# DataCanvasIO/DeepTables

Measured on AMD Instinct MI355X. Metric: training rows/sec (fwd+bwd) DeepFM Criteo-shape batch 8192, higher is better.
Workload: dtype f32 (split-bf16: 24-bit fwd / 16-bit bwd)

## Files before the change

__graft_entry__.py:

```python
import glob
import hashlib
import os
import subprocess
import sys

ROOT = os.path.dirname(os.path.abspath(__file__))
CSRC = os.path.join(ROOT, 'deeptables_amd', 'csrc')
LIB = os.path.join(ROOT, 'deeptables_amd', 'libdt_hip.so')


def _sources():
    return sorted(glob.glob(os.path.join(CSRC, '*.hip')) + glob.glob(os.path.join(CSRC, '*.cpp')))


def _deps():
    return _sources() + sorted(glob.glob(os.path.join(CSRC, '*.h'))) + [os.path.join(ROOT, 'include', 'dt_hip.h')]


def source_hash():
    h = hashlib.sha256()
    for p in _deps():
        h.update(os.path.basename(p).encode())
        h.update(open(p, 'rb').read())
    return h.hexdigest()[:16]


def _loaded_hash():
    if not os.path.exists(LIB):
        return None
    code = ('import ctypes,sys; l=ctypes.CDLL(sys.argv[1]); f=l.dt_source_hash; f.restype=ctypes.c_char_p; '
            'print(f().decode())')
    try:
        return subprocess.check_output([sys.executable, '-c', code, LIB], stderr=subprocess.DEVNULL,
                                       timeout=60).decode().strip()
    except Exception:
        return None


def _compile_one(args):
    hipcc, src, obj, want = args
    cmd = [hipcc, '--offload-arch=gfx950', '-O3', '-std=c++17', '-fPIC', '-Wno-unused-value',
           f'-DDT_SOURCE_HASH="{want}"' if src.endswith('lib.cpp') else '-DDT_UNUSED', '-x', 'hip', '-c', src, '-o', obj]
    subprocess.check_call(cmd)
    return obj


def build(force=False):
    want = source_hash()
    have = None if force else _loaded_hash()
    if have != want:
        hipcc = os.environ.get('HIPCC', '/opt/rocm/bin/hipcc')
        if not os.path.exists(hipcc):
            raise RuntimeError(f'hipcc not found and the in-tree libdt_hip.so ({have}) does not match the sources ({want})')
        bdir = os.path.join(CSRC, '_build')
        os.makedirs(bdir, exist_ok=True)
        common = hashlib.sha256()
        for p in _deps():
            if p.endswith('.h'):
                common.update(open(p, 'rb').read())
        jobs, objs = [], []
        for src in _sources():
            key = hashlib.sha256(common.digest() + open(src, 'rb').read() +
                                 (want.encode() if src.endswith('lib.cpp') else b'')).hexdigest()[:16]
            obj = os.path.join(bdir, os.path.basename(src) + '.' + key + '.o')
            objs.append(obj)
            if force or not os.path.exists(obj):
                for old in glob.glob(os.path.join(bdir, os.path.basename(src) + '.*.o')):
                    os.remove(old)
                jobs.append((hipcc, src, obj, want))
        print(f'[build] hipcc --offload-arch=gfx950 -O3: {len(jobs)} of {len(objs)} objects to compile')
        if jobs:
            from concurrent.futures import ThreadPoolExecutor
            with ThreadPoolExecutor(max_workers=min(len(jobs), os.cpu_count() or 4)) as ex:
                list(ex.map(_compile_one, jobs))
        subprocess.check_call([hipcc, '--offload-arch=gfx950', '-shared', '-fPIC'] + objs + ['-o', LIB + '.tmp'])
        os.replace(LIB + '.tmp', LIB)
    if ROOT not in sys.path:
        sys.path.insert(0, ROOT)
    import deeptables_amd
    from deeptables_amd import _lib
    h = _lib.lib()
    assert h.dt_version() == 1 and h.dt_build_arch() == b'gfx950'
    got = h.dt_source_hash().decode()
    assert got == want, f'libdt_hip.so was built from other sources: {got} != {want}'
    print('[build] ok:', LIB, 'exports', len(_lib.SIGNATURES), 'entry points; source hash', got,
          '(rebuilt)' if have != want else '(binary matches the sources)')


def smoke():
    if ROOT not in sys.path:
        sys.path.insert(0, ROOT)
    build()
    import torch
    assert torch.cuda.is_available(), 'smoke() needs a GPU'
    from deeptables_amd import functional, ops
    from deeptables_amd.models import ModelConfig, DeepModel, deepnets
    from deeptables_amd.models.metainfo import CategoricalColumn, ContinuousColumn
    from oracle import bridge, reference_layers as R
    dev = torch.device('cuda', 0)
    F, Nd, D, B, V = 26, 13, 16, 256, 1000
    functional.set_seed(7)
    conf = ModelConfig(nets=deepnets.DeepFM, fixed_embedding_dim=True, embeddings_output_dim=D,
                       embedding_dropout=0, metrics=['AUC'])
    cats = [CategoricalColumn(f'C{i}', V, D) for i in range(F)]
    conts = [ContinuousColumn('input_continuous_all', [f'I{j}' for j in range(Nd)])]
    dm = DeepModel('binary', 2, conf, cats, conts)
    dm.build(dev)
    g = torch.Generator().manual_seed(1)
    idx = torch.randint(0, V, (B, F), generator=g)
    dense = torch.randn(B, Nd, generator=g)
    y = (torch.rand(B, 1, generator=g) < 0.25).float()
    ref_logit, _ = bridge.oracle_forward(dm, idx, dense, training=True)
    dm.model.train()
    emb_layer = dm.model.layers_by_name['emb_categorical_vars_all']
    emb, _ = ops.embedding_lookup(idx.int().to(dev), emb_layer.tables['d16'], emb_layer.row_offset_d16,
                                  emb_layer.vocab_d16)
    ref_emb = torch.cat(R.multi_column_embedding(idx.float(), [e.detach().cpu() for e in emb_layer.embeddings]), 1)
    assert torch.equal(emb.detach().cpu(), ref_emb), 'embedding gather is not bit-exact'
    loss, logit = dm.train_step([idx.int().to(dev), dense.to(dev)], y.to(dev))
    torch.cuda.synchronize()
    err = (logit.double().cpu() - ref_logit).abs().max().item()
    print(f'[smoke] DeepFM B={B}: loss={float(loss):.6f}  max|logit - oracle|={err:.2e}  gather bit-exact')
    assert err < 1e-4, f'logit mismatch vs oracle: {err}'


if __name__ == '__main__':
    build(force='--force' in sys.argv)
    if '--smoke' in sys.argv:
        smoke()
```

deeptables_amd/csrc/deepfm.hip:

```cpp
#include <stdlib.h>
#include "common.h"
#include "adam_dev.h"

namespace dt {

typedef float floatx16 __attribute__((ext_vector_type(16)));
typedef float floatx4_t __attribute__((ext_vector_type(4)));

constexpr int kH1 = 128;
constexpr int kH2 = 64;
constexpr int kTM = 32;

struct DeepFmDims {
    int B, F, D, Nd, C, CP;
};

struct DeepFmAccum {
    int64_t dW1, dW2, db1, db2, dw3, dwo, dbo, loss, dgamma, dbeta, dwlin, slin, total;
    int64_t dw3d, dcw, dcb, sumc, sumcx;
};
__host__ __device__ inline DeepFmAccum deepfm_accum_layout(int C, int CP, int F, int Nd, int L = 0) {
    DeepFmAccum a;
    int64_t o = 0;
    a.dW1 = o; o += (int64_t)C * kH1;
// ... 1771 lines not shown
#pragma unroll
            for (int pt = 0; pt < 2; ++pt) {
                lay.W2R[pt * lay.w2r_lo + (int64_t)k0 * kH2 + n] = q0[pt];
                lay.W2R[pt * lay.w2r_lo + (int64_t)(k0 + 1) * kH2 + n] = q1[pt];
            }
        }
        return;
    }
    const float dg = wave_sum(w.x * m.x + w.y * m.y);
    const float db = wave_sum(w.x * d.x + w.y * d.y);
    const float ga_b = ga, be_b = be;
    {
        const floatx2 g = floatx2{ga * m.x + be * d.x, ga * m.y + be * d.y};
        *reinterpret_cast<floatx2*>(accum + e0) = g;
        if (da.p) adam2(g.x, g.y);
        if (da.p && lay.W1B) {
            __bf16 q0[3], q1[3];
            x3_parts(pnew[0], q0);
            x3_parts(pnew[1], q1);
            const int k = col, n0 = 2 * lane;
            const int64_t kb = ((int64_t)(k >> 5) * 8) * 64 * 8 + (((k >> 3) & 3) * 16) * 8 + (k & 7);
            const int64_t i0 = kb + ((int64_t)(n0 >> 4) * 64 + (n0 & 15)) * 8, i1 = kb + ((int64_t)((n0 + 1) >> 4) * 64 + ((n0 + 1) & 15)) * 8;
#pragma unroll
            for (int pt = 0; pt < 3; ++pt) {
                lay.W1B[pt * lay.w1b_lo + i0] = q0[pt];
                lay.W1B[pt * lay.w1b_lo + i1] = q1[pt];
            }
#pragma unroll
            for (int pt = 0; pt < 2; ++pt) {
                typedef __bf16 b2 __attribute__((ext_vector_type(2)));
                *reinterpret_cast<b2*>(lay.W1R + pt * lay.w1r_lo + (int64_t)k * kH1 + n0) = b2{q0[pt], q1[pt]};
            }
        }
    }
    if (Lc) {
        const int scal = pl.cross + (Lc + 1) * dm.CP;
        const int l = lane;
        const float sa_mine = l < Lc ? rec_sum(rs, scal + 16 + l) : 0.f;
        const float sco_mine = l <= Lc ? rec_sum(rs, scal + l) : 0.f;
        const float G = l <= Lc ? gp.gsum[(int64_t)l * dm.CP + col] : 0.f;
        const float sdz = rec_sum(rs, scal + 31);
        float cl = 0.f, suf = 0.f;
        for (int j = 0; j < Lc; ++j) {
            const float saj = __shfl(sa_mine, j, 64);
            const float bj = cb[(int64_t)j * dm.C + col], wj = cw[(int64_t)j * dm.C + col];
            if (j < l) cl += bj;
            if (j > l) suf += saj * wj;
        }
        if (l <= Lc) {
            const int64_t ig = l < Lc ? al.dcw + (int64_t)l * dm.C + col : al.dw3 + col;
            const float gw = ga_b * G + be_b * sco_mine + (l < Lc ? sa_mine : sdz) * cl;
            const float gb = sdz * w3c[col] + suf;
            accum[ig] = gw;
            if (l < Lc) accum[al.dcb + (int64_t)l * dm.C + col] = gb;
            if (da.p) {
                adam_one(da.p, da.m, da.v, ig, gw, da.lr_t, da.b1, da.b2, da.eps);
                if (l < Lc) adam_one(da.p, da.m, da.v, al.dcb + (int64_t)l * dm.C + col, gb, da.lr_t, da.b1, da.b2, da.eps);
                if (lay.cwp) {
                    lay.cwp[(int64_t)(l < Lc ? l : 2 * Lc) * dm.CP + col] = da.p[ig];
                    if (l < Lc) lay.cwp[(int64_t)(Lc + l) * dm.CP + col] = da.p[al.dcb + (int64_t)l * dm.C + col];
                }
            }
        }
    }
}

__global__ __launch_bounds__(256) void k_bn_grads2(const float* __restrict__ W1, const float* __restrict__ gamma,
                                                   const float* __restrict__ beta, DeepFmDims dm, float* accum,
                                                   DeepFmAccum al, const float* __restrict__ wpart, int row_blocks,
                                                   int Lc, const float* __restrict__ cw, const float* __restrict__ cb,
                                                   const float* __restrict__ w3c, RecSrc rs, int col_blocks, GPart gp) {
    __shared__ floatx2 sm[4][64];
    __shared__ float slin_s[kMaxC];
    const DenseAdam none{nullptr, nullptr, nullptr, 0.f, 0.f, 0.f, 0.f};
    const Part3 pl = part3_layout(dm.CP, Lc, 1);
    if ((int)blockIdx.x < col_blocks)
        bn_grads2_body(W1, gamma, beta, dm, accum, al, wpart, row_blocks, Lc, cw, cb, w3c, rs, pl, sm, slin_s, none, (int)blockIdx.x, gp);
    else
        finish_record_entry(((int)blockIdx.x - col_blocks) * (int)blockDim.x + (int)threadIdx.x, rs, pl, al, dm, Lc, accum, none);
}

__global__ __launch_bounds__(256) void k_finish_records(DeepFmDims dm, float* accum, DeepFmAccum al, int Lc, RecSrc rs,
                                                        double* __restrict__ bnacc_zero, int bnacc_n) {
    const DenseAdam none{nullptr, nullptr, nullptr, 0.f, 0.f, 0.f, 0.f};
    const Part3 pl = part3_layout(dm.CP, Lc, 0);
    const int i = (int)blockIdx.x * (int)blockDim.x + (int)threadIdx.x;
    finish_record_entry(i, rs, pl, al, dm, Lc, accum, none);
    for (int j = i; j < bnacc_n; j += (int)(gridDim.x * blockDim.x)) bnacc_zero[j] = 0.0;
}

struct FinishSeg {
    SegTail seg;
    float *table, *m, *v;
    const float* values;
    int sstride, D;
};
__global__ __launch_bounds__(256) void k_finish_step(const float* __restrict__ W1, const float* __restrict__ gamma,
                                                     const float* __restrict__ beta, DeepFmDims dm, float* accum,
                                                     DeepFmAccum al, const float* __restrict__ wpart, int row_blocks,
                                                     DenseAdam da, AdamState* __restrict__ st, float lr, int col_blocks,
                                                     int small_blocks, int seg_blocks, FinishSeg fs, int Lc,
                                                     const float* __restrict__ cw, const float* __restrict__ cb,
                                                     const float* __restrict__ w3c, RecSrc rs, X3Lay lay, GPart gp,
                                                     const float* __restrict__ lr_snap) {
    __shared__ floatx2 sm[4][64];
    __shared__ float slin_s[kMaxC];
    const Part3 pl = part3_layout(dm.CP, Lc, 1);
    const int sb = (int)blockIdx.x < seg_blocks ? (int)blockIdx.x : -1;
    const int b = sb >= 0 ? col_blocks + small_blocks : (int)blockIdx.x - seg_blocks < small_blocks
                      ? col_blocks + ((int)blockIdx.x - seg_blocks) : (int)blockIdx.x - seg_blocks - small_blocks;
    int nseg0 = 0;
    if (sb >= 0 && fs.seg.nseg) nseg0 = fs.seg.nseg[(sb * (int)(blockDim.x >> 6) + (int)(threadIdx.x >> 6)) % fs.seg.regions];
    if (lr_snap) da.lr_t = *lr_snap; else if (st) da.lr_t = st->lr_t;
    if (b < col_blocks) {
        bn_grads2_body(W1, gamma, beta, dm, accum, al, wpart, row_blocks, Lc, cw, cb, w3c, rs, pl, sm, slin_s, da, b, gp, lay);
    } else if (b < col_blocks + small_blocks) {
        finish_record_entry((b - col_blocks) * (int)blockDim.x + (int)threadIdx.x, rs, pl, al, dm, Lc, accum, da);
    } else if (fs.seg.nseg) {
        adam_segments<true>(fs.seg, seg_blocks, nseg0, fs.table, fs.m, fs.v, fs.values, fs.D, da.lr_t, da.b1, da.b2, da.eps,
                      fs.sstride, sb);
    }
    if (lr_snap) {
        if (blockIdx.x == 0 && threadIdx.x == 0 && st) {
            const int t = st->t + 1;
            st->t = t;
            st->lr_t = adam_lr_t(lr, da.b1, da.b2, t);
        }
    } else {
        __syncthreads();
        adam_finish(st, threadIdx.x == 0 ? 0u : kNoTicket, lr, da.b1, da.b2);
    }
}

__global__ void k_emb_drop_advance(unsigned* seed) { *seed = *seed * 1664525u + 1013904223u; }

struct RowsAdam {
    float *table, *m, *v;
    int sstride;
    const float* lr_t_dev;
    float lr_t_host, b1, b2, eps;
    int wt;
};
struct RowsEpi {
    const float *dXn, *X, *dz, *S, *wlin, *sc, *mean, *rstd;
    RecSrc rs;
    int sdx, sdxx;
    const int64_t* rows_out;
    float* grad_rows;
    float grad_scale;
    int field_major;
};
constexpr int kRowsUB = 4;

template <bool DCN>
__device__ __forceinline__ void rows_epilogue_wave(unsigned* work, int first_tile, int tile_stride, const DeepFmDims& dm,
                                                   const RowsEpi& a, const RowsAdam& ad, const EmbDrop& drop) {
    const int lane = threadIdx.x & 63, wv = threadIdx.x >> 6;
    const int LPR = dm.D >> 2, TPR = dm.F * LPR;
    const int parts = TPR > 64 ? 2 : 1;
    const int lpp = (TPR + parts - 1) / parts;
    const int rpw = parts == 1 ? 64 / TPR : 1;
    const int part = wv & (parts - 1);
    const int rsub = lane / lpp, pl = lane - rsub * lpp;
    const int piece = min(part * lpp + pl, TPR - 1);
    const bool active = rsub < rpw && part * lpp + pl < TPR;
    const int f = piece / LPR, c = piece - f * LPR;
    const int col = 4 * piece;
    const int tiles = (dm.B + kTM - 1) / kTM;
    const int chunk_rows = rpw * kRowsUB, chunks = (kTM + chunk_rows - 1) / chunk_rows;
    int dshift = 0;
    while ((1 << dshift) < dm.D) ++dshift;
    const floatx4 ca = ld4(a.sc + col), cmu = ld4(a.mean + col);
    floatx4 c1, c2;
    {
        typedef double doublex2 __attribute__((ext_vector_type(2)));
        doublex2 s1[2] = {{0.0, 0.0}, {0.0, 0.0}}, s2[2] = {{0.0, 0.0}, {0.0, 0.0}};
#pragma unroll
        for (int sh = 0; sh < kRecShards; ++sh) {
            const double* q = a.rs.racc + (int64_t)sh * a.rs.stride;
            s1[0] += *reinterpret_cast<const doublex2*>(q + a.sdx + col);
            s1[1] += *reinterpret_cast<const doublex2*>(q + a.sdx + col + 2);
            s2[0] += *reinterpret_cast<const doublex2*>(q + a.sdxx + col);
            s2[1] += *reinterpret_cast<const doublex2*>(q + a.sdxx + col + 2);
        }
        const floatx4 rsd = ld4(a.rstd + col);
        const float invN = 1.0f / (float)dm.B;
        c1 = floatx4{(float)s1[0][0], (float)s1[0][1], (float)s1[1][0], (float)s1[1][1]} * invN;
        c2 = rsd * floatx4{(float)s2[0][0], (float)s2[0][1], (float)s2[1][0], (float)s2[1][1]} * invN;
    }
    const float wl = DCN ? 0.f : a.wlin[f];
    const float lr_t = ad.lr_t_dev ? *ad.lr_t_dev : ad.lr_t_host;
    const unsigned dseed = drop.thr ? *drop.seed : 0u;
    for (;;) {
        unsigned it = 0;
        if (lane == 0) it = atomicAdd(&work[part], 1u);
        it = __builtin_amdgcn_readfirstlane(it);
        const int ti = (int)(it / (unsigned)chunks), ch = (int)(it - (unsigned)ti * (unsigned)chunks);
        const int tile = first_tile + ti * tile_stride;
        if (tile >= tiles) break;
        const int b0 = tile * kTM;
        {
            int64_t row[kRowsUB];
            floatx4 gx[kRowsUB], xr[kRowsUB], sv[kRowsUB];
            float dzv[kRowsUB];
            bool ok[kRowsUB];
            int bb[kRowsUB];
#pragma unroll
            for (int k = 0; k < kRowsUB; ++k) {
                const int r = ch * chunk_rows + k * rpw + rsub;
                ok[k] = active && r < kTM && b0 + r < dm.B;
                bb[k] = min(b0 + min(r, kTM - 1), dm.B - 1);
                row[k] = a.rows_out[(int64_t)bb[k] * dm.F + f];
            }
#pragma unroll
            for (int k = 0; k < kRowsUB; ++k) {
                gx[k] = ld4(a.dXn + (int64_t)bb[k] * dm.CP + col);
                xr[k] = ld4(a.X + (int64_t)bb[k] * dm.CP + col);
                if (!DCN) {
                    sv[k] = ld4(a.S + ((int64_t)bb[k] << dshift) + 4 * c);
                    dzv[k] = a.dz[bb[k]];
                }
            }
            floatx4 pv[kRowsUB], mv[kRowsUB], vv[kRowsUB];
            bool upd[kRowsUB];
#pragma unroll
            for (int k = 0; k < kRowsUB; ++k) {
                upd[k] = ok[k] && ad.table && row[k] >= 0;
                if (ad.table) {
                    const int64_t rr = upd[k] ? row[k] : 0;
                    pv[k] = drop.thr ? ld4(ad.table + (rr << dshift) + 4 * c) : xr[k];
                    mv[k] = ld4(ad.m + rr * ad.sstride + 4 * c);
                    vv[k] = ld4(ad.v + rr * ad.sstride + 4 * c);
                }
            }
#pragma unroll
            for (int k = 0; k < kRowsUB; ++k) {
                floatx4 g = ca * (gx[k] - c1 - (xr[k] - cmu) * c2);
                if (!DCN) g = g + dzv[k] * wl + dzv[k] * (sv[k] - xr[k]);
                if (drop.thr) {
                    float4 t4 = make_float4(g.x, g.y, g.z, g.w);
                    t4 = emb_drop4(t4, dseed, drop.thr, drop.inv_keep, (unsigned)bb[k], (unsigned)col);
                    g = floatx4{t4.x, t4.y, t4.z, t4.w};
                }
                if (upd[k]) {
                    floatx4 mi = mv[k], vi = vv[k], pi = pv[k];
#pragma unroll
                    for (int e = 0; e < 4; ++e) {
                        mi[e] = ad.b1 * mi[e] + (1.f - ad.b1) * g[e];
                        vi[e] = ad.b2 * vi[e] + (1.f - ad.b2) * g[e] * g[e];
                        pi[e] -= lr_t * mi[e] / (sqrtf(vi[e]) + ad.eps);
                    }
                    st4_sel(ad.m + row[k] * ad.sstride + 4 * c, mi, ad.wt);
                    st4_sel(ad.v + row[k] * ad.sstride + 4 * c, vi, ad.wt);
                    st4_sel(ad.table + (row[k] << dshift) + 4 * c, pi, ad.wt);
                } else if (ok[k]) {
                    if (a.field_major)
                        st4(a.grad_rows + (((int64_t)f * dm.B + bb[k]) << dshift) + 4 * c, g * a.grad_scale);
                    else
                        st4(a.grad_rows + (((int64_t)bb[k] * dm.F + f) << dshift) + 4 * c, g);
                }
            }
        }
    }
}

template <bool DCN, int WM = 0>
__global__ __launch_bounds__(512) void k_wgrad_rows(const float* __restrict__ X, MlpParams p, DeepFmDims dm,
                                                    const float* __restrict__ H1, const float* __restrict__ dH1,
                                                    const float* __restrict__ dH2, int row_blocks, int rows_per_block,
                                                    float* __restrict__ wpart, unsigned long long* stamps_all,
                                                    RowsEpi ep, RowsAdam ad, EmbDrop drop,
                                                    unsigned long long* stamps_rows, int matrix_waves_join,
                                                    double* __restrict__ bnacc_zero, int bnacc_n, StepNext nx, GPart gp,
                                                    float* __restrict__ lr_snap) {
    extern __shared__ __attribute__((aligned(16))) float red[];
    __shared__ unsigned arrived, work[2], ecnt;
    if (threadIdx.x == 0) { arrived = 0u; work[0] = 0u; work[1] = 0u; ecnt = 0u; }
    __syncthreads();
    if (threadIdx.x < 256) {
        if constexpr (WM == 0)
            wgrad_heavy(red, (int)blockIdx.x, X, p, dm, H1, dH1, dH2, row_blocks, rows_per_block, wpart, stamps_all, &arrived);
        else
            wgrad_heavy_bf16<WM>(red, (int)blockIdx.x, X, p, dm, H1, dH1, dH2, row_blocks, rows_per_block, wpart, &arrived);
        ElectSync sy{&ecnt, 0u};
        if (DCN && gp.part) reduce_gpart(gp, red, (int)blockIdx.x, (int)gridDim.x, (int)threadIdx.x, sy);
        if (nx.idx) {
            for (int e = (int)blockIdx.x; e < nx.eblocks; e += (int)gridDim.x) {
                elect_barrier<256, true>(sy);
                elect_block<256, true, 32>(reinterpret_cast<unsigned long long*>(red), nx.dd, dm.B, dm.F, e, (int)threadIdx.x,
                                           nx.rows_out, sy);
            }
        }
        if (matrix_waves_join) rows_epilogue_wave<DCN>(work, (int)blockIdx.x, (int)gridDim.x, dm, ep, ad, drop);
        if (stamps_all && threadIdx.x == 0) stamps_all[(int64_t)blockIdx.x * 16 + 6] = __builtin_amdgcn_s_memtime();
    } else {
        if (stamps_rows && threadIdx.x == 256) stamps_rows[(int64_t)blockIdx.x * 16] = __builtin_amdgcn_s_memtime();
        for (int j = (int)blockIdx.x * 256 + ((int)threadIdx.x - 256); j < bnacc_n; j += (int)gridDim.x * 256) bnacc_zero[j] = 0.0;
        if (lr_snap && blockIdx.x == 0 && threadIdx.x == 256) *lr_snap = ad.lr_t_dev ? *ad.lr_t_dev : ad.lr_t_host;
        rows_epilogue_wave<DCN>(work, (int)blockIdx.x, (int)gridDim.x, dm, ep, ad, drop);
        if (stamps_rows && threadIdx.x == 256) stamps_rows[(int64_t)blockIdx.x * 16 + 3] = __builtin_amdgcn_s_memtime();
    }
}

}

using namespace dt;

static bool deepfm_dims(int B, int F, int D, int Nd, DeepFmDims* dm, int* lpr) {
    if (B <= 0 || F <= 0 || D <= 0 || Nd < 0 || D % 4) return false;
    const int l = D / 4;
    if (l < 1 || l > 64 || (l & (l - 1))) return false;
    if (F * l > 128 || Nd > 64) return false;
    dm->B = B; dm->F = F; dm->D = D; dm->Nd = Nd;
    dm->C = F * D + Nd;
    dm->CP = (dm->C + 63) & ~63;
    if (dm->C > 544 || D > 64) return false;
    *lpr = l;
    return true;
}

extern "C" int dt_deepfm_supported(int B, int F, int D, int Nd, int H1, int H2) {
    DeepFmDims dm; int lpr;
    return (H1 == kH1 && H2 == kH2 && deepfm_dims(B, F, D, Nd, &dm, &lpr)) ? 1 : 0;
}

struct DeepFmWs {
    int64_t X, H1, dH1, dH2, lin, fm, z, dz, dlogit, mean, rstd, sc, betap, W1L, W2L, W2TL, S, wpart, bnacc, racc, stamps, dXc, dXn,
        gammap, x3, total;
    int64_t bnacc_n, racc_n;
    int64_t gpart, gsum;
    int64_t lrsnap;
};
static DeepFmWs deepfm_ws_layout(const DeepFmDims& dm, int L = 0) {
    DeepFmWs w;
    int64_t o = 0;
    auto take = [&](int64_t n) { int64_t r = o; o += (n + 3) & ~(int64_t)3; return r; };
    const int tiles = ceil_div(dm.B, kTM);
    const int64_t rows = (int64_t)tiles * kTM;
    w.X = take(rows * dm.CP);
    w.H1 = take(rows * kH1);
    w.dH1 = take(rows * kH1);
    w.dH2 = take(rows * kH2);
    w.lin = take(rows); w.fm = take(rows); w.z = take(rows); w.dz = take(rows); w.dlogit = take(rows);
    w.mean = take(dm.CP); w.rstd = take(dm.CP); w.sc = take(dm.CP); w.betap = take(dm.CP);
    w.W1L = take((int64_t)dm.CP * kH1);
    w.W2L = take((int64_t)kH1 * kH2);
    w.W2TL = take((int64_t)kH1 * kH2);
    w.S = take(rows * dm.D);
    w.wpart = take((int64_t)256 * 8192);
    w.bnacc_n = (int64_t)kBnShards * 2 * dm.CP;
    w.bnacc = take(2 * w.bnacc_n);
    w.racc_n = (int64_t)kRecShards * part3_layout(dm.CP, L, 1).stride;
    w.racc = take(2 * w.racc_n);
    w.gpart = take(L > 0 ? (int64_t)tiles * (L + 1) * dm.CP : 0);
    w.gsum = take(L > 0 ? (int64_t)(L + 1) * dm.CP : 0);
    w.stamps = take((int64_t)5 * tiles * 16 * 2);
    w.dXc = take(L > 0 ? rows * dm.CP : 0);
    w.dXn = take(rows * dm.CP);
    w.gammap = take(dm.CP);
    w.lrsnap = take(4);
    w.x3 = take((5 * (int64_t)dm.CP * kH1 + 5 * (int64_t)kH1 * kH2 + 1) / 2 + (2 * kCrossMax + 1) * (int64_t)dm.CP);
    w.total = o;
    return w;
}

extern "C" int64_t dt_deepfm_workspace_bytes(int B, int F, int D, int Nd) {
    DeepFmDims dm; int lpr;
    if (!deepfm_dims(B, F, D, Nd, &dm, &lpr)) return -1;
    return deepfm_ws_layout(dm).total * (int64_t)sizeof(float);
}

extern "C" int64_t dt_deepfm_stamps_offset_floats(int B, int F, int D, int Nd) {
    DeepFmDims dm; int lpr;
    if (!deepfm_dims(B, F, D, Nd, &dm, &lpr)) return -1;
    return deepfm_ws_layout(dm).stamps;
}

extern "C" int64_t dt_deepfm_accum_floats(int F, int D, int Nd) {
    const int C = F * D + Nd, CP = (C + 63) & ~63;
    return deepfm_accum_layout(C, CP, F, Nd).total;
}

extern "C" int dt_deepfm_accum_offsets(int F, int D, int Nd, int64_t* out11) {
    const int C = F * D + Nd, CP = (C + 63) & ~63;
    const DeepFmAccum a = deepfm_accum_layout(C, CP, F, Nd);
    const int64_t v[11] = {a.dW1, a.dW2, a.db1, a.db2, a.dw3, a.dwo, a.dbo, a.loss, a.dgamma, a.dbeta, a.dwlin};
    for (int i = 0; i < 11; ++i) out11[i] = v[i];
    return DT_OK;
}

extern "C" unsigned dt_deepfm_dropout_hash(unsigned seed, unsigned b, unsigned col) { return emb_drop_hash(seed, b, col); }

extern "C" int64_t dt_deepfm_dedupe_slots(int B, int F) {
    return (int64_t)B * F;
}

struct DedupeLayout {
    int64_t rows_fm, nseg, seg_row, seg_off, seg_cnt, seg_list, list_cur, overflow, pid, total;
    int pid_stride;
    int eblocks, parts_log2;
    int regions, cap;
    bool by_field;
};
static DedupeLayout dedupe_layout(int B, int F) {
    const int64_t n = (int64_t)B * F;
    DedupeLayout l;
    l.by_field = B > kElectSlots;
    l.parts_log2 = 0;
    while (((l.by_field ? 4096 : 1024) << l.parts_log2) < B) ++l.parts_log2;
    const int fpad = ((F + 7) >> 3) << 3;
    l.eblocks = fpad << l.parts_log2;
    l.regions = l.by_field ? fpad : l.eblocks;
    l.cap = l.by_field ? (B >> 1) : kSegCap;
    int64_t o = 0;
    auto take = [&](int64_t bytes) { int64_t r = o; o += (bytes + 15) & ~(int64_t)15; return r; };
    l.rows_fm = take(n * 8); l.nseg = take((int64_t)l.regions * 4);
    l.seg_row = take((int64_t)l.regions * l.cap * 8); l.seg_off = take((int64_t)l.regions * l.cap * 4);
    l.seg_cnt = take((int64_t)l.regions * l.cap * 4); l.seg_list = take((int64_t)l.regions * B * 4);
    l.list_cur = take((int64_t)fpad * 4);
    l.overflow = take(16);
    l.pid_stride = (B + 15) & ~15;
    l.pid = take(l.by_field ? (int64_t)fpad * l.pid_stride : 0);
    l.total = o;
    return l;
}
static DedupeWs dedupe_view(void* dedupe_ws, const DedupeLayout& dl) {
    char* base = reinterpret_cast<char*>(dedupe_ws);
    DedupeWs dd{reinterpret_cast<int64_t*>(base + dl.rows_fm), dl.parts_log2, reinterpret_cast<int*>(base + dl.nseg),
                reinterpret_cast<int64_t*>(base + dl.seg_row), reinterpret_cast<int*>(base + dl.seg_off),
                reinterpret_cast<int*>(base + dl.seg_cnt), reinterpret_cast<int*>(base + dl.seg_list),
                dl.by_field ? reinterpret_cast<int*>(base + dl.nseg) : nullptr,
                dl.by_field ? reinterpret_cast<int*>(base + dl.list_cur) : nullptr,
                reinterpret_cast<int*>(base + dl.overflow),
                dl.by_field ? reinterpret_cast<unsigned char*>(base + dl.pid) : nullptr, dl.pid_stride};
    return dd;
}

extern "C" int64_t dt_deepfm_dedupe_bytes(int B, int F) { return dedupe_layout(B, F).total; }

extern "C" int dt_deepfm_dedupe_segments(int B, int F, int64_t* out7) {
    const DedupeLayout l = dedupe_layout(B, F);
    out7[0] = l.nseg; out7[1] = l.seg_row; out7[2] = l.seg_off; out7[3] = l.seg_cnt; out7[4] = l.seg_list;
    out7[5] = l.regions; out7[6] = l.cap;
    return DT_OK;
}

extern "C" int64_t dt_deepfm_dedupe_overflow_offset(int B, int F) { return dedupe_layout(B, F).overflow; }

extern "C" int dt_deepfm_preelect(const void* idx, int idx_kind, const int64_t* row_offset, const int32_t* vocab, int B,
                                  int F, int64_t* rows_out, void* dedupe_ws, int64_t dedupe_slots, void* stream) {
    DT_REQUIRE(idx && row_offset && vocab && rows_out && dedupe_ws && B > 0 && F > 0 && F <= 128,
               "dt_deepfm_preelect: bad arguments");
// ... 639 lines not shown
```

deeptables_amd/csrc/tower_x3.h:

```cpp
#pragma once

typedef __bf16 x3_b8 __attribute__((ext_vector_type(8)));
typedef __bf16 x3_b4 __attribute__((ext_vector_type(4)));

struct X3Weights {
    const __bf16* W1B; int64_t w1b_lo;
    const __bf16* W1R; int64_t w1r_lo;
    const __bf16* W2B; int64_t w2b_lo;
    const __bf16* W2R; int64_t w2r_lo;
    const float* cwp;
};

__device__ __forceinline__ void x3_split2(const float (&v)[8], x3_b8& h, x3_b8& l) {
#pragma unroll
    for (int e = 0; e < 8; ++e) {
        const __bf16 a = (__bf16)v[e];
        h[e] = a;
        l[e] = (__bf16)(v[e] - (float)a);
    }
}
__device__ __forceinline__ void x3_split3(const float (&v)[8], x3_b8& h, x3_b8& m, x3_b8& l) {
#pragma unroll
    for (int e = 0; e < 8; ++e) {
        const __bf16 a = (__bf16)v[e];
// ... 25 lines not shown
}

template <int NCH, int LC = 0, bool ONE = false>
__global__ __launch_bounds__(512) void k_tower_x3(const float* __restrict__ X, MlpParams p, X3Weights xw, DeepFmDims dm,
                                                  const float* __restrict__ lin, const float* __restrict__ fm,
                                                  const float* __restrict__ y, float* __restrict__ H1,
                                                  float* __restrict__ dH1, float* __restrict__ dH2,
                                                  float* __restrict__ z_out, float* __restrict__ logit_out,
                                                  float* __restrict__ dlogit, float* __restrict__ dz_out,
                                                  double* __restrict__ part, unsigned long long* stamps, DcnArgs dc,
                                                  float* __restrict__ dxn_out) {
    extern __shared__ __attribute__((aligned(16))) float lds[];
    DT_STAMP(stamps, 0);
    constexpr int CP = 64 * NCH, NST = CP / 32, XSB = CP + 16, XS = CP + 4, HF = kH1 + 4, DF = kH2 + 4;
    constexpr int XP = kTM * XSB;
    char* base = reinterpret_cast<char*>(lds);
    __bf16* xb = reinterpret_cast<__bf16*>(base);
    float* xs = reinterpret_cast<float*>(base);
    float* slp = xs + kTM * XS;
    float* zp = slp + 8 * CP;
    float* dzs = zp + 4 * kTM;
    float* cs = dzs + kTM;
    float* bnp = reinterpret_cast<float*>(base + (size_t)3 * XP * 2);
    float* h1f = bnp + 4 * CP;
    float* d2f = h1f + kTM * HF;
    float* pb = d2f + kTM * DF;
    float* crP = pb + 2 * 48 * 16;
    float* crA = crP + 48 * 16;
    float* crF = crA + kTM * 16;
    float* zcs = crF + kTM * 16;
    const int tid = threadIdx.x, lane = tid & 63, wave = tid >> 6;
    const int n16 = lane & 15, kg = lane >> 4;
    const int m0 = blockIdx.x * kTM;
    const Part3 pl = part3_layout(dm.CP, LC ? dc.L : 0, 1);
    double* prec = part + (int64_t)((int)blockIdx.x & (kRecShards - 1)) * pl.stride;

    const int srow = tid >> 4, qcol = 4 * (tid & 15);
    const int bcol = min(tid, dm.C - 1);
    double bsx[kBnShards], bsq[kBnShards];
#pragma unroll
    for (int w = 0; w < kBnShards; ++w) {
        bsx[w] = p.bnacc[(int64_t)w * 2 * dm.CP + bcol];
        bsq[w] = p.bnacc[(int64_t)w * 2 * dm.CP + dm.CP + bcol];
    }
    const float gam = p.gamma[bcol], bet = p.beta[bcol];
    floatx4 xv[NCH];
#pragma unroll
    for (int j = 0; j < NCH; ++j) xv[j] = ld4(X + (int64_t)(m0 + srow) * CP + 64 * j + qcol);
    constexpr int kPF = 5;
    const __bf16* w1b = xw.W1B + ((int64_t)wave * 64 + lane) * 8;
    x3_b8 bq[kPF][3];
#pragma unroll
    for (int s = 0; s < kPF; ++s)
#pragma unroll
        for (int q = 0; q < 3; ++q) bq[s][q] = x3_ld8(w1b + q * xw.w1b_lo + (int64_t)(s < NST ? s : 0) * 4096);
    const int mt2 = wave & 1, nt2 = wave >> 1;
    const float bias1 = p.b1[16 * wave + n16];
    const float b2v = p.b2[16 * nt2 + n16], w3v = p.w3[16 * nt2 + n16];
    float linv = 0.f, fmv = 0.f, yv = 0.f, wov = 0.f, bov = 0.f, swv = 1.f;
    const float invB = 1.0f / (float)dm.B;
    const double invBd = 1.0 / (double)dm.B;
    if (wave == 0) {
        wov = p.wo[0];
        bov = p.bo ? p.bo[0] : 0.f;
        if (lane < 32 && m0 + lane < dm.B) {
            if (LC == 0) { linv = lin[m0 + lane]; fmv = fm[m0 + lane]; }
            yv = y[m0 + lane];
            if (dc.sw) swv = dc.sw[m0 + lane];
        }
    }
    DT_STAMP(stamps, 6);
    {
        const int col = tid;
        float mean = 0.f, sc = 0.f, be = 0.f, rstd = 0.f, var = 0.f;
        if (col < dm.C) {
            double sx = 0.0, sq = 0.0;
#pragma unroll
            for (int w = 0; w < kBnShards; ++w) { sx += bsx[w]; sq += bsq[w]; }
            const double md = sx * invBd, vd = sq * invBd - md * md;
            mean = (float)md;
            var = vd > 0.0 ? (float)vd : 0.f;
            rstd = 1.0f / sqrtf(var + p.eps);
            sc = rstd * gam;
            be = bet;
        }
        if (col < CP) {
            bnp[col] = mean; bnp[CP + col] = sc; bnp[2 * CP + col] = be; bnp[3 * CP + col] = rstd;
            if (blockIdx.x == 0) {
                p.mean_w[col] = mean; p.rstd_w[col] = rstd; p.sc_w[col] = sc; p.betap_w[col] = be;
                p.gammap_w[col] = col < dm.C ? gam : 0.f;
                if (col < dm.C) {
                    if (p.moving_mean) p.moving_mean[col] = p.moving_mean[col] * p.momentum + mean * (1.f - p.momentum);
                    if (p.moving_var) p.moving_var[col] = p.moving_var[col] * p.momentum + var * (1.f - p.momentum);
                }
            }
        }
    }
    static_assert(CP <= 512, "one column per thread in the BN prologue");
    lds_barrier();
    DT_STAMP(stamps, 7);
#pragma unroll
    for (int j = 0; j < NCH; ++j) {
        const floatx4 mu = ld4(bnp + 64 * j + qcol), sc = ld4(bnp + CP + 64 * j + qcol), be = ld4(bnp + 2 * CP + 64 * j + qcol);
        const floatx4 xn = (xv[j] - mu) * sc + be;
        x3_b4 h, m, l;
#pragma unroll
        for (int e = 0; e < 4; ++e) {
            const __bf16 a = (__bf16)xn[e];
            const float r1 = xn[e] - (float)a;
            const __bf16 b = (__bf16)r1;
            h[e] = a; m[e] = b; l[e] = (__bf16)(r1 - (float)b);
        }
        __bf16* dst = xb + srow * XSB + 64 * j + qcol;
        *reinterpret_cast<x3_b4*>(dst) = h;
        *reinterpret_cast<x3_b4*>(dst + XP) = m;
        *reinterpret_cast<x3_b4*>(dst + 2 * XP) = l;
    }
    lds_barrier();
    DT_STAMP(stamps, 1);

    x3_b8 w2q[4][3];
    float h1r[2][4];
    {
        floatx4 c1[2], c2[2], c3[2];
#pragma unroll
        for (int t = 0; t < 2; ++t) { c1[t] = floatx4{0.f, 0.f, 0.f, 0.f}; c2[t] = c1[t]; c3[t] = c1[t]; }
        const __bf16* arow0 = xb + n16 * XSB + 8 * kg;
        const __bf16* arow1 = xb + (16 + n16) * XSB + 8 * kg;
        x3_b8 an[2][3];
#pragma unroll
        for (int q = 0; q < 3; ++q) { an[0][q] = x3_ld8(arow0 + q * XP); an[1][q] = x3_ld8(arow1 + q * XP); }
#pragma unroll
        for (int s = 0; s < NST; ++s) {
            x3_b8 a[2][3], b[3];
#pragma unroll
            for (int q = 0; q < 3; ++q) { a[0][q] = an[0][q]; a[1][q] = an[1][q]; b[q] = bq[s % kPF][q]; }
            if (s + 1 < NST) {
#pragma unroll
                for (int q = 0; q < 3; ++q) {
                    an[0][q] = x3_ld8(arow0 + q * XP + 32 * (s + 1));
                    an[1][q] = x3_ld8(arow1 + q * XP + 32 * (s + 1));
                }
            }
            if (s + kPF < NST) {
#pragma unroll
                for (int q = 0; q < 3; ++q) bq[s % kPF][q] = x3_ld8(w1b + q * xw.w1b_lo + (int64_t)(s + kPF) * 4096);
            }
            if (NST >= 4 && s >= NST - 4) {
                const int g = s - (NST - 4);
                const __bf16* w2b = xw.W2B + (((int64_t)g * 4 + nt2) * 64 + lane) * 8;
#pragma unroll
                for (int q = 0; q < 3; ++q) w2q[g][q] = x3_ld8(w2b + q * xw.w2b_lo);
            }
            X3_MFMA(c1[0], a[0][0], b[0]); X3_MFMA(c1[1], a[1][0], b[0]);
            X3_LO(c2[0], a[0][0], b[1]); X3_LO(c2[1], a[1][0], b[1]);
            X3_LO(c3[0], a[0][0], b[2]); X3_LO(c3[1], a[1][0], b[2]);
            X3_LO(c2[0], a[0][1], b[0]); X3_LO(c2[1], a[1][1], b[0]);
            X3_LO(c3[0], a[0][1], b[1]); X3_LO(c3[1], a[1][1], b[1]);
            X3_LO(c3[0], a[0][2], b[0]); X3_LO(c3[1], a[1][2], b[0]);
        }
        if constexpr (NST < 4) {
#pragma unroll
            for (int g = 0; g < 4; ++g) {
                const __bf16* w2b = xw.W2B + (((int64_t)g * 4 + nt2) * 64 + lane) * 8;
#pragma unroll
                for (int q = 0; q < 3; ++q) w2q[g][q] = x3_ld8(w2b + q * xw.w2b_lo);
            }
        }
        DT_STAMP(stamps, 2);
        if constexpr (LC > 0) {
            if (wave < 6) {
                const int L = dc.L, mt = wave % 3, kh = wave / 3;
                const int s0 = kh * (NST / 2), s1 = kh ? NST : NST / 2;
                const float* brow = xw.cwp + (int64_t)(n16 < L ? n16 : 2 * L) * CP + 8 * kg;
                const float bmask = n16 <= L ? 1.f : 0.f;
                const float* arow2 = xw.cwp + (int64_t)(L + min(n16, L - 1)) * CP + 8 * kg;
                const float amask2 = n16 < L ? 1.f : 0.f;
                floatx4 q1 = {0.f, 0.f, 0.f, 0.f}, q2 = q1, q3 = q1;
                for (int st = s0; st < s1; ++st) {
                    float bv[8];
                    x3_ld8f(brow + 32 * st, bv);
#pragma unroll
                    for (int e = 0; e < 8; ++e) bv[e] *= bmask;
                    x3_b8 b1, b2, b3, a1, a2, a3;
                    x3_split3(bv, b1, b2, b3);
                    if (mt < 2) {
                        const __bf16* ap = xb + (16 * mt + n16) * XSB + 32 * st + 8 * kg;
                        a1 = x3_ld8(ap); a2 = x3_ld8(ap + XP); a3 = x3_ld8(ap + 2 * XP);
                    } else {
                        float av[8];
                        x3_ld8f(arow2 + 32 * st, av);
#pragma unroll
                        for (int e = 0; e < 8; ++e) av[e] *= amask2;
                        x3_split3(av, a1, a2, a3);
                    }
                    X3_MFMA(q3, a1, b3); X3_MFMA(q3, a2, b2); X3_MFMA(q3, a3, b1);
                    X3_MFMA(q2, a1, b2); X3_MFMA(q2, a2, b1);
                    X3_MFMA(q1, a1, b1);
                }
#pragma unroll
                for (int r = 0; r < 4; ++r) pb[(kh * 48 + 16 * mt + 4 * kg + r) * 16 + n16] = (q3[r] + q2[r]) + q1[r];
            }
        }
#pragma unroll
        for (int t = 0; t < 2; ++t)
#pragma unroll
            for (int r = 0; r < 4; ++r) {
                const float h = fmaxf(((c3[t][r] + c2[t][r]) + c1[t][r]) + bias1, 0.f);
                h1r[t][r] = h;
                h1f[(16 * t + 4 * kg + r) * HF + 16 * wave + n16] = h;
            }
    }
    x3_b8 w2r[2][2];
#pragma unroll
    for (int g = 0; g < 2; ++g) {
        const __bf16* src = xw.W2R + (int64_t)(16 * wave + n16) * kH2 + 32 * g + 8 * kg;
        w2r[g][0] = x3_ld8(src); w2r[g][1] = x3_ld8(src + xw.w2r_lo);
    }
    lds_barrier();
    DT_STAMP(stamps, 3);

    float h2r[4];
    {
        floatx4 c1 = {0.f, 0.f, 0.f, 0.f}, c2 = c1, c3 = c1;
        const float* arow = h1f + (16 * mt2 + n16) * HF + 8 * kg;
        floatx4 hrow[2];
#pragma unroll
        for (int u = 0; u < 2; ++u) hrow[u] = ld4(h1f + ((tid >> 5) + 16 * u) * HF + 4 * (tid & 31));
#pragma unroll
        for (int g = 0; g < 4; ++g) {
            float v[8];
            x3_ld8f(arow + 32 * g, v);
            x3_b8 a1, a2, a3;
            x3_split3(v, a1, a2, a3);
            X3_MFMA(c1, a1, w2q[g][0]);
            X3_LO(c2, a1, w2q[g][1]);
            X3_LO(c3, a1, w2q[g][2]);
            X3_LO(c2, a2, w2q[g][0]);
            X3_LO(c3, a2, w2q[g][1]);
            X3_LO(c3, a3, w2q[g][0]);
        }
#pragma unroll
        for (int u = 0; u < 2; ++u) {
            const int m = m0 + (tid >> 5) + 16 * u;
            if (m < dm.B) st4_sel(H1 + (int64_t)m * kH1 + 4 * (tid & 31), hrow[u], dc.wt);
        }
        float zr[4];
#pragma unroll
        for (int r = 0; r < 4; ++r) {
            h2r[r] = fmaxf(((c3[r] + c2[r]) + c1[r]) + b2v, 0.f);
            zr[r] = group_sum<16>(h2r[r] * w3v);
        }
        if (n16 == 0) {
#pragma unroll
            for (int r = 0; r < 4; ++r) zp[nt2 * kTM + 16 * mt2 + 4 * kg + r] = zr[r];
        }
    }
#pragma unroll
    for (int j = 0; j < NCH; ++j) {
        const floatx4 mu = ld4(bnp + 64 * j + qcol), rs = ld4(bnp + 3 * CP + 64 * j + qcol);
        st4(xs + srow * XS + 64 * j + qcol, (xv[j] - mu) * rs);
    }
    if constexpr (LC > 0) {
        for (int e = tid; e < 48 * 16; e += 512) crP[e] = pb[e] + pb[48 * 16 + e];
    }
    lds_barrier();
    DT_STAMP(stamps, 4);
    const int NT = (dm.C + 15) >> 4;
    auto w1r = [&](int nt) {
        const int col = min(16 * nt + n16, CP - 1);
        return xw.W1R + (int64_t)col * kH1 + 8 * kg;
    };
    x3_b8 bW[2][4][2];
#pragma unroll
    for (int i = 0; i < 2; ++i) {
        if (wave + 8 * i < NT) {
            const __bf16* wr = w1r(wave + 8 * i);
#pragma unroll
            for (int g = 0; g < 4; ++g) { bW[i][g][0] = x3_ld8(wr + 32 * g); bW[i][g][1] = x3_ld8(wr + xw.w1r_lo + 32 * g); }
        }
    }

    if (wave == 0) {
        const int c = lane & 31, s = lane >> 5;
        const int m = m0 + c;
        float zc = 0.f;
        if constexpr (LC > 0) {
            const int L = dc.L;
            static_assert(LC + 1 <= 12, "three float4 per row of crP");
            float pr[12], gq[LC][12];
            {
                const floatx4 t0 = ld4(crP + c * 16), t1 = ld4(crP + c * 16 + 4), t2 = ld4(crP + c * 16 + 8);
#pragma unroll
                for (int e = 0; e < 4; ++e) { pr[e] = t0[e]; pr[4 + e] = t1[e]; pr[8 + e] = t2[e]; }
            }
#pragma unroll
            for (int j = 0; j < LC; ++j) {
                const floatx4 t0 = ld4(crP + (32 + j) * 16), t1 = ld4(crP + (32 + j) * 16 + 4), t2 = ld4(crP + (32 + j) * 16 + 8);
#pragma unroll
                for (int e = 0; e < 4; ++e) { gq[j][e] = t0[e]; gq[j][4 + e] = t1[e]; gq[j][8 + e] = t2[e]; }
            }
            float a = 1.f;
#pragma unroll
            for (int l = 0; l <= LC; ++l) {
                float q = 0.f;
#pragma unroll
// ... 45 lines not shown

    {
        float sb = 0.f, sw = 0.f;
#pragma unroll
        for (int r = 0; r < 4; ++r) {
            const int row = 16 * mt2 + 4 * kg + r;
            const float dzv = dzs[row];
            const float g = h2r[r] > 0.f ? dzv * w3v : 0.f;
            d2f[row * DF + 16 * nt2 + n16] = g;
            sb += g;
            sw += dzv * h2r[r];
        }
        sb = row_pair16(sb, false); sw = row_pair16(sw, false);
        if (kg == 0) { cs[(mt2 * 2 + 0) * kH2 + 16 * nt2 + n16] = sb; cs[(mt2 * 2 + 1) * kH2 + 16 * nt2 + n16] = sw; }
        if constexpr (LC == 0) {
            const float dzr = dzs[srow];
#pragma unroll
            for (int j = 0; j < NCH; ++j) {
                floatx4 v = xv[j] * dzr;
#pragma unroll
                for (int e = 0; e < 4; ++e) v[e] = row_pair16(v[e], false);
                if (kg == 0) st4(slp + wave * CP + 64 * j + qcol, v);
            }
        } else if (wave == 7 && lane < kTM) {
            const int L = dc.L, r = lane;
            float pr[12], av[12];
            {
                const floatx4 t0 = ld4(crP + r * 16), t1 = ld4(crP + r * 16 + 4), t2 = ld4(crP + r * 16 + 8);
                const floatx4 u0 = ld4(crA + r * 16), u1 = ld4(crA + r * 16 + 4), u2 = ld4(crA + r * 16 + 8);
#pragma unroll
                for (int e = 0; e < 4; ++e) {
                    pr[e] = t0[e]; pr[4 + e] = t1[e]; pr[8 + e] = t2[e];
                    av[e] = u0[e]; av[4 + e] = u1[e]; av[8 + e] = u2[e];
                }
            }
            const float dzv = dzs[r];
            float pL = 0.f, aL = 0.f;
#pragma unroll
            for (int l = 0; l <= LC; ++l) { pL = l == L ? pr[l] : pL; aL = l == L ? av[l] : aL; }
            float cf[16], sa[16];
#pragma unroll
            for (int l = 0; l < 16; ++l) { cf[l] = 0.f; sa[l] = 0.f; }
            float A = dzv * pL;
#pragma unroll
            for (int l = LC - 1; l >= 0; --l) {
                if (l < L) {
                    cf[l] = A * av[l];
                    sa[l] = A;
                    A *= 1.f + pr[l];
                }
            }
#pragma unroll
            for (int l = 0; l <= LC; ++l) cf[l] = l == L ? dzv * aL : cf[l];
            sa[15] = dzv;
#pragma unroll
            for (int e = 0; e < 4; ++e) {
                st4(crF + r * 16 + 4 * e, floatx4{cf[4 * e], cf[4 * e + 1], cf[4 * e + 2], cf[4 * e + 3]});
                st4(crA + r * 16 + 4 * e, floatx4{sa[4 * e], sa[4 * e + 1], sa[4 * e + 2], sa[4 * e + 3]});
            }
        }
    }
    lds_barrier();
    DT_STAMP(stamps, 9);

    {
        floatx4 dH[2], dM[2];
#pragma unroll
        for (int t = 0; t < 2; ++t) { dH[t] = floatx4{0.f, 0.f, 0.f, 0.f}; dM[t] = dH[t]; }
        const floatx4 drow = ld4(d2f + (tid >> 4) * DF + 4 * (tid & 15));
#pragma unroll
        for (int g = 0; g < 2; ++g)
#pragma unroll
            for (int t = 0; t < 2; ++t) {
                float v[8];
                x3_ld8f(d2f + (16 * t + n16) * DF + 32 * g + 8 * kg, v);
                x3_b8 ah, al;
                x3_split2(v, ah, al);
                X3_MFMA(dH[t], ah, w2r[g][0]);
                X3_LO(dM[t], ah, w2r[g][1]);
                X3_LO(dM[t], al, w2r[g][0]);
            }
        if (tid < kH2) {
            radd(prec + pl.db2 + tid, cs[tid] + cs[2 * kH2 + tid]);
            radd(prec + pl.dw3 + tid, cs[kH2 + tid] + cs[3 * kH2 + tid]);
        }
        {
            const int m = m0 + (tid >> 4);
            if (m < dm.B) st4_sel(dH2 + (int64_t)m * kH2 + 4 * (tid & 15), drow, dc.wt);
        }
        if constexpr (LC == 0) {
            for (int col = tid; col < CP; col += 512) {
                float v = 0.f;
#pragma unroll
                for (int w = 0; w < 8; ++w) v += slp[w * CP + col];
                radd(prec + pl.slin + col, v);
            }
        } else {
            const int L = dc.L;
            double* rec = prec + pl.cross;
            const float* crS = crA;
            if (wave == 7) {
                floatx4 d1 = {0.f, 0.f, 0.f, 0.f}, d2 = d1;
#pragma unroll
                for (int st = 0; st < 8; ++st) {
                    d1 = __builtin_amdgcn_mfma_f32_16x16x4f32(1.f, crF[(4 * st + kg) * 16 + n16], d1, 0, 0, 0);
                    d2 = __builtin_amdgcn_mfma_f32_16x16x4f32(1.f, crS[(4 * st + kg) * 16 + n16], d2, 0, 0, 0);
                }
                if (kg == 0) { radd(rec + (L + 1) * CP + n16, d1[0]); radd(rec + (L + 1) * CP + 16 + n16, d2[0]); }
            }
            float bop[8];
#pragma unroll
            for (int st = 0; st < 8; ++st) bop[st] = crF[(4 * st + kg) * 16 + n16];
            for (int ct = wave; ct < 4 * NCH; ct += 8) {
                floatx4 d = {0.f, 0.f, 0.f, 0.f};
#pragma unroll
                for (int st = 0; st < 8; ++st)
                    d = __builtin_amdgcn_mfma_f32_16x16x4f32(xs[(4 * st + kg) * XS + 16 * ct + n16], bop[st], d, 0, 0, 0);
                if (n16 <= L) {
                    st4(dc.gpart + (int64_t)blockIdx.x * dc.gstride + n16 * CP + 16 * ct + 4 * kg, d);
                }
            }
        }
        float colsum = 0.f;
#pragma unroll
        for (int t = 0; t < 2; ++t)
#pragma unroll
            for (int r = 0; r < 4; ++r) {
                const float g = h1r[t][r] > 0.f ? dH[t][r] + dM[t][r] : 0.f;
                h1f[(16 * t + 4 * kg + r) * HF + 16 * wave + n16] = g;
                colsum += g;
            }
        colsum = row_pair16(colsum, false);
        if (kg == 0) radd(prec + pl.db1 + 16 * wave + n16, colsum);
    }
    lds_barrier();
    DT_STAMP(stamps, 8);

    {
        x3_b8 ah[2][4], al[2][4];
#pragma unroll
        for (int t = 0; t < 2; ++t)
#pragma unroll
            for (int g = 0; g < 4; ++g) {
                float v[8];
                x3_ld8f(h1f + (16 * t + n16) * HF + 32 * g + 8 * kg, v);
                x3_split2(v, ah[t][g], al[t][g]);
            }
#pragma unroll
        for (int u = 0; u < 2; ++u) {
            const int r = (tid >> 5) + 16 * u;
            if (m0 + r < dm.B) st4_sel(dH1 + (int64_t)(m0 + r) * kH1 + 4 * (tid & 31), ld4(h1f + r * HF + 4 * (tid & 31)), dc.wt);
        }
        DT_STAMP(stamps, 13);
        auto tile = [&](int buf, int nt) {
            floatx4 gH[2], gM[2];
#pragma unroll
            for (int t = 0; t < 2; ++t) { gH[t] = floatx4{0.f, 0.f, 0.f, 0.f}; gM[t] = gH[t]; }
            const int col = 16 * nt + n16;
            float xh_[2][4];
#pragma unroll
            for (int t = 0; t < 2; ++t)
#pragma unroll
                for (int r = 0; r < 4; ++r) xh_[t][r] = xs[(16 * t + 4 * kg + r) * XS + col];
#pragma unroll
            for (int g = 0; g < 4; ++g) {
                X3_MFMA(gH[0], ah[0][g], bW[buf][g][0]); X3_MFMA(gH[1], ah[1][g], bW[buf][g][0]);
                X3_LO(gM[0], ah[0][g], bW[buf][g][1]); X3_LO(gM[1], ah[1][g], bW[buf][g][1]);
                X3_LO(gM[0], al[0][g], bW[buf][g][0]); X3_LO(gM[1], al[1][g], bW[buf][g][0]);
            }
            if constexpr (LC > 0) {
                const int L = dc.L;
#pragma unroll
                for (int g2 = 0; g2 < 4; ++g2) {
                    const int l = 4 * g2 + kg;
                    const float bw = l <= L ? xw.cwp[(int64_t)(l < L ? l : 2 * L) * CP + col] : 0.f;
                    gH[0] = __builtin_amdgcn_mfma_f32_16x16x4f32(crF[n16 * 16 + l], bw, gH[0], 0, 0, 0);
                    gH[1] = __builtin_amdgcn_mfma_f32_16x16x4f32(crF[(16 + n16) * 16 + l], bw, gH[1], 0, 0, 0);
                }
            }
            if (nt + 16 < NT) {
                const __bf16* wn = w1r(nt + 16);
#pragma unroll
                for (int g = 0; g < 4; ++g) { bW[buf][g][0] = x3_ld8(wn + 32 * g); bW[buf][g][1] = x3_ld8(wn + xw.w1r_lo + 32 * g); }
            }
            float s1 = 0.f, s2 = 0.f;
#pragma unroll
            for (int t = 0; t < 2; ++t)
#pragma unroll
                for (int r = 0; r < 4; ++r) {
                    const float gx = gH[t][r] + gM[t][r];
                    s1 += gx;
                    s2 += gx * xh_[t][r];
                    xs[(16 * t + 4 * kg + r) * XS + col] = gx;
                }
            s1 = row_pair16(s1, false); s2 = row_pair16(s2, false);
            if (kg == 0 && col < dm.C) { radd(prec + pl.sdx + col, s1); radd(prec + pl.sdxx + col, s2); }
        };
        if (wave < NT) tile(0, wave);
        if (wave + 8 < NT) tile(1, wave + 8);
        if (wave + 16 < NT) tile(0, wave + 16);
        if (wave + 24 < NT) tile(1, wave + 24);
    }
    lds_barrier();
    DT_STAMP(stamps, 14);
    {
        const int fq = (dm.F * dm.D) >> 2;
        const int rgs = 512 / fq, rg = tid / fq, q = tid - rg * fq;
        if (rg < rgs) {
            for (int row = rg; row < kTM; row += rgs)
                if (m0 + row < dm.B) st4_sel(dxn_out + (int64_t)(m0 + row) * CP + 4 * q, ld4(xs + row * XS + 4 * q), dc.wt);
        }
    }
    DT_STAMP(stamps, 15);
}
```

Baseline: 82.79 million.

## Specialize row epilogue on table/dropout and restructure tower backward tile loop

Templates the rows epilogue on whether an Adam table is present and whether embedding dropout is active, so runtime branches are resolved at compile time via a small dispatcher. Restructures the tower backward tile loop to dispatch on a compile-time tile count, removes the runtime prefetch-bound checks, and defers the per-column reduction atomics until after all tiles. Adds sched_barrier hints to constrain instruction scheduling around the MFMA blocks and uses explicit FMAs. The aim is less branching and register pressure in hot kernels, at the cost of more template instantiations and code size, with the sched barriers possibly hurting latency hiding.

Result: faster. 84.39 million (median of 6 runs) (+1.9%).

```diff
diff --git a/__graft_entry__.py b/__graft_entry__.py
--- a/__graft_entry__.py
+++ b/__graft_entry__.py
@@ -37,9 +37,12 @@
         return None
 
 
+HIPCC_FLAGS = ['--offload-arch=gfx950', '-O3', '-std=c++17', '-fPIC', '-Wno-unused-value']
+
+
 def _compile_one(args):
     hipcc, src, obj, want = args
-    cmd = [hipcc, '--offload-arch=gfx950', '-O3', '-std=c++17', '-fPIC', '-Wno-unused-value',
+    cmd = [hipcc] + HIPCC_FLAGS + [
            f'-DDT_SOURCE_HASH="{want}"' if src.endswith('lib.cpp') else '-DDT_UNUSED', '-x', 'hip', '-c', src, '-o', obj]
     subprocess.check_call(cmd)
     return obj
diff --git a/deeptables_amd/csrc/deepfm.hip b/deeptables_amd/csrc/deepfm.hip
--- a/deeptables_amd/csrc/deepfm.hip
+++ b/deeptables_amd/csrc/deepfm.hip
@@ -1947,7 +1947,7 @@
 };
 constexpr int kRowsUB = 4;
 
-template <bool DCN>
+template <bool DCN, bool TABLE, int DROP>
 __device__ __forceinline__ void rows_epilogue_wave(unsigned* work, int first_tile, int tile_stride, const DeepFmDims& dm,
                                                    const RowsEpi& a, const RowsAdam& ad, const EmbDrop& drop) {
     const int lane = threadIdx.x & 63, wv = threadIdx.x >> 6;
@@ -1985,7 +1985,8 @@
     }
     const float wl = DCN ? 0.f : a.wlin[f];
     const float lr_t = ad.lr_t_dev ? *ad.lr_t_dev : ad.lr_t_host;
-    const unsigned dseed = drop.thr ? *drop.seed : 0u;
+    const bool dropping = DROP < 0 ? drop.thr != 0u : DROP == 1;
+    const unsigned dseed = dropping ? *drop.seed : 0u;
     for (;;) {
         unsigned it = 0;
         if (lane == 0) it = atomicAdd(&work[part], 1u);
@@ -2020,10 +2021,10 @@
             bool upd[kRowsUB];
 #pragma unroll
             for (int k = 0; k < kRowsUB; ++k) {
-                upd[k] = ok[k] && ad.table && row[k] >= 0;
-                if (ad.table) {
+                upd[k] = TABLE && ok[k] && row[k] >= 0;
+                if constexpr (TABLE) {
                     const int64_t rr = upd[k] ? row[k] : 0;
-                    pv[k] = drop.thr ? ld4(ad.table + (rr << dshift) + 4 * c) : xr[k];
+                    pv[k] = DROP == 1 ? ld4(ad.table + (rr << dshift) + 4 * c) : xr[k];
                     mv[k] = ld4(ad.m + rr * ad.sstride + 4 * c);
                     vv[k] = ld4(ad.v + rr * ad.sstride + 4 * c);
                 }
@@ -2032,19 +2033,22 @@
             for (int k = 0; k < kRowsUB; ++k) {
                 floatx4 g = ca * (gx[k] - c1 - (xr[k] - cmu) * c2);
                 if (!DCN) g = g + dzv[k] * wl + dzv[k] * (sv[k] - xr[k]);
-                if (drop.thr) {
+                if (dropping) {
                     float4 t4 = make_float4(g.x, g.y, g.z, g.w);
                     t4 = emb_drop4(t4, dseed, drop.thr, drop.inv_keep, (unsigned)bb[k], (unsigned)col);
                     g = floatx4{t4.x, t4.y, t4.z, t4.w};
                 }
-                if (upd[k]) {
-                    floatx4 mi = mv[k], vi = vv[k], pi = pv[k];
+                floatx4 mi = {0.f, 0.f, 0.f, 0.f}, vi = mi, pi = mi;
+                if constexpr (TABLE) {
+                    mi = mv[k]; vi = vv[k]; pi = pv[k];
 #pragma unroll
                     for (int e = 0; e < 4; ++e) {
-                        mi[e] = ad.b1 * mi[e] + (1.f - ad.b1) * g[e];
-                        vi[e] = ad.b2 * vi[e] + (1.f - ad.b2) * g[e] * g[e];
+                        mi[e] = __builtin_fmaf(ad.b1, mi[e], (1.f - ad.b1) * g[e]);
+                        vi[e] = __builtin_fmaf(ad.b2, vi[e], (1.f - ad.b2) * g[e] * g[e]);
                         pi[e] -= lr_t * mi[e] / (sqrtf(vi[e]) + ad.eps);
                     }
+                }
+                if (upd[k]) {
                     st4_sel(ad.m + row[k] * ad.sstride + 4 * c, mi, ad.wt);
                     st4_sel(ad.v + row[k] * ad.sstride + 4 * c, vi, ad.wt);
                     st4_sel(ad.table + (row[k] << dshift) + 4 * c, pi, ad.wt);
@@ -2057,6 +2061,14 @@
             }
         }
     }
+}
+
+template <bool DCN>
+__device__ __forceinline__ void rows_epilogue(unsigned* work, int first_tile, int tile_stride, const DeepFmDims& dm,
+                                              const RowsEpi& a, const RowsAdam& ad, const EmbDrop& drop) {
+    if (!ad.table) rows_epilogue_wave<DCN, false, -1>(work, first_tile, tile_stride, dm, a, ad, drop);
+    else if (drop.thr) rows_epilogue_wave<DCN, true, 1>(work, first_tile, tile_stride, dm, a, ad, drop);
+    else rows_epilogue_wave<DCN, true, 0>(work, first_tile, tile_stride, dm, a, ad, drop);
 }
 
 template <bool DCN, int WM = 0>
@@ -2086,13 +2098,13 @@
                                            nx.rows_out, sy);
             }
         }
-        if (matrix_waves_join) rows_epilogue_wave<DCN>(work, (int)blockIdx.x, (int)gridDim.x, dm, ep, ad, drop);
+        if (matrix_waves_join) rows_epilogue<DCN>(work, (int)blockIdx.x, (int)gridDim.x, dm, ep, ad, drop);
         if (stamps_all && threadIdx.x == 0) stamps_all[(int64_t)blockIdx.x * 16 + 6] = __builtin_amdgcn_s_memtime();
     } else {
         if (stamps_rows && threadIdx.x == 256) stamps_rows[(int64_t)blockIdx.x * 16] = __builtin_amdgcn_s_memtime();
         for (int j = (int)blockIdx.x * 256 + ((int)threadIdx.x - 256); j < bnacc_n; j += (int)gridDim.x * 256) bnacc_zero[j] = 0.0;
         if (lr_snap && blockIdx.x == 0 && threadIdx.x == 256) *lr_snap = ad.lr_t_dev ? *ad.lr_t_dev : ad.lr_t_host;
-        rows_epilogue_wave<DCN>(work, (int)blockIdx.x, (int)gridDim.x, dm, ep, ad, drop);
+        rows_epilogue<DCN>(work, (int)blockIdx.x, (int)gridDim.x, dm, ep, ad, drop);
         if (stamps_rows && threadIdx.x == 256) stamps_rows[(int64_t)blockIdx.x * 16 + 3] = __builtin_amdgcn_s_memtime();
     }
 }
diff --git a/deeptables_amd/csrc/tower_x3.h b/deeptables_amd/csrc/tower_x3.h
--- a/deeptables_amd/csrc/tower_x3.h
+++ b/deeptables_amd/csrc/tower_x3.h
@@ -201,6 +201,7 @@
 #pragma unroll
                 for (int q = 0; q < 3; ++q) w2q[g][q] = x3_ld8(w2b + q * xw.w2b_lo);
             }
+            __builtin_amdgcn_sched_barrier(0);
             X3_MFMA(c1[0], a[0][0], b[0]); X3_MFMA(c1[1], a[1][0], b[0]);
             X3_LO(c2[0], a[0][0], b[1]); X3_LO(c2[1], a[1][0], b[1]);
             X3_LO(c3[0], a[0][0], b[2]); X3_LO(c3[1], a[1][0], b[2]);
@@ -552,7 +553,8 @@
             if (m0 + r < dm.B) st4_sel(dH1 + (int64_t)(m0 + r) * kH1 + 4 * (tid & 31), ld4(h1f + r * HF + 4 * (tid & 31)), dc.wt);
         }
         DT_STAMP(stamps, 13);
-        auto tile = [&](int buf, int nt) {
+        float cs1[4], cs2[4];
+        auto tile = [&](int buf, int nt, int k, bool pf) {
             floatx4 gH[2], gM[2];
 #pragma unroll
             for (int t = 0; t < 2; ++t) { gH[t] = floatx4{0.f, 0.f, 0.f, 0.f}; gM[t] = gH[t]; }
@@ -578,11 +580,12 @@
                     gH[1] = __builtin_amdgcn_mfma_f32_16x16x4f32(crF[(16 + n16) * 16 + l], bw, gH[1], 0, 0, 0);
                 }
             }
-            if (nt + 16 < NT) {
+            if (pf) {
                 const __bf16* wn = w1r(nt + 16);
 #pragma unroll
                 for (int g = 0; g < 4; ++g) { bW[buf][g][0] = x3_ld8(wn + 32 * g); bW[buf][g][1] = x3_ld8(wn + xw.w1r_lo + 32 * g); }
             }
+            __builtin_amdgcn_sched_barrier(0);
             float s1 = 0.f, s2 = 0.f;
 #pragma unroll
             for (int t = 0; t < 2; ++t)
@@ -590,16 +593,33 @@
                 for (int r = 0; r < 4; ++r) {
                     const float gx = gH[t][r] + gM[t][r];
                     s1 += gx;
-                    s2 += gx * xh_[t][r];
+                    s2 = __builtin_fmaf(gx, xh_[t][r], s2);
                     xs[(16 * t + 4 * kg + r) * XS + col] = gx;
                 }
-            s1 = row_pair16(s1, false); s2 = row_pair16(s2, false);
-            if (kg == 0 && col < dm.C) { radd(prec + pl.sdx + col, s1); radd(prec + pl.sdxx + col, s2); }
+            cs1[k] = row_pair16(s1, false); cs2[k] = row_pair16(s2, false);
         };
-        if (wave < NT) tile(0, wave);
-        if (wave + 8 < NT) tile(1, wave + 8);
-        if (wave + 16 < NT) tile(0, wave + 16);
-        if (wave + 24 < NT) tile(1, wave + 24);
+        const int nw = wave < NT ? min((NT - 1 - wave) / 8 + 1, 4) : 0;
+        auto tiles = [&](auto n_) {
+            constexpr int n = decltype(n_)::value;
+            tile(0, wave, 0, n > 2);
+            if constexpr (n > 1) tile(1, wave + 8, 1, n > 3);
+            if constexpr (n > 2) tile(0, wave + 16, 2, false);
+            if constexpr (n > 3) tile(1, wave + 24, 3, false);
+        };
+        switch (nw) {
+            case 4: tiles(std::integral_constant<int, 4>{}); break;
+            case 3: tiles(std::integral_constant<int, 3>{}); break;
+            case 2: tiles(std::integral_constant<int, 2>{}); break;
+            case 1: tiles(std::integral_constant<int, 1>{}); break;
+            default: break;
+        }
+        if (kg == 0) {
+#pragma unroll
+            for (int k = 0; k < 4; ++k) {
+                const int col = 16 * (wave + 8 * k) + n16;
+                if (k < nw && col < dm.C) { radd(prec + pl.sdx + col, cs1[k]); radd(prec + pl.sdxx + col, cs2[k]); }
+            }
+        }
     }
     lds_barrier();
     DT_STAMP(stamps, 14);
```
